# jiwoon-ahn/irn

Hardware: NVIDIA H100
Metric: pseudo-label images/sec (CAM+random-walk) (higher is better)
Workload: dtype f32

## Files before the change

irn_b200/csrc/conv_wgmma.cuh:

```cuda
#pragma once
#include <cuda.h>
#include <cuda_runtime.h>
#include <cstdint>
#include <type_traits>

#include "tma.cuh"

namespace irn {

constexpr int kTcTW = 16, kTcTH = 8;
constexpr int kTcBK = 32;
constexpr int kBfBK = 64;
constexpr int kWgThreads = 384;

struct TcMaps {
    CUtensorMap a;
    CUtensorMap b_hi;
    CUtensorMap b_lo;
    CUtensorMap a2;
};

struct TcArgs {
    const float* bias;
    const float* residual;
    float* out;
    int B, Ho, Wo, Cout, Cin, ksize, stride, pad, relu;
    int tiles_x, tiles_y;
    int kb_split = 1 << 30;
    int stride2 = 1;
    const float* oscale = nullptr;
    int stem = 0;
};

template <bool F16, int BN>
struct WgCfg {
    static constexpr int kBK = F16 ? kBfBK : kTcBK;
    static constexpr int kARaw = F16 ? 32768 : 16384;
    static constexpr int kBBytes = BN * 128;
    static constexpr int kStageBytes = kARaw + 2 * kBBytes;
    static constexpr int kMaxSmem = 227 * 1024;
    static constexpr int kBarBytes = 256;
    static constexpr int kStages = (kMaxSmem - 1024 - kBarBytes) / kStageBytes;
    static constexpr size_t kSmem = 1024 + (size_t)kStages * kStageBytes + kBarBytes;
    static_assert(kStages >= 2, "shared memory holds at least two stages");
    static_assert(2 * kStages * 8 <= kBarBytes, "barrier area holds full[S] and empty[S]");
    static_assert(BN == 64 || BN == 128, "N tile 64 or 128");
};
constexpr int kWgProducerRegs = 40, kWgConsumerRegs = 232;

#ifdef __CUDACC__
__device__ __forceinline__ uint64_t wg_desc(uint32_t smem_addr) {
    return (uint64_t)((smem_addr & 0x3FFFFu) >> 4) | ((uint64_t)1 << 16) | ((uint64_t)(1024 >> 4) << 32) | ((uint64_t)1 << 62);
}
__device__ __forceinline__ void wg_fence() { asm volatile("wgmma.fence.sync.aligned;" ::: "memory"); }
__device__ __forceinline__ void wg_commit() { asm volatile("wgmma.commit_group.sync.aligned;" ::: "memory"); }
template <int N>
__device__ __forceinline__ void wg_wait() { asm volatile("wgmma.wait_group.sync.aligned %0;" ::"n"(N) : "memory"); }
template <int N>
__device__ __forceinline__ void setmaxnreg_inc() { asm volatile("setmaxnreg.inc.sync.aligned.u32 %0;" ::"n"(N)); }
template <int N>
__device__ __forceinline__ void setmaxnreg_dec() { asm volatile("setmaxnreg.dec.sync.aligned.u32 %0;" ::"n"(N)); }
template <int N>
__device__ __forceinline__ void wg_fence_regs(float (&d)[N]) {
#pragma unroll
    for (int i = 0; i < N; ++i) asm volatile("" : "+f"(d[i])::"memory");
}

template <bool F16, int N>
__device__ __forceinline__ void wg_mma(float (&d)[N / 2], const uint32_t (&a)[4], uint64_t db, uint32_t scale_d);

template <> __device__ __forceinline__ void wg_mma<false, 64>(float (&d)[32], const uint32_t (&a)[4], uint64_t db, uint32_t scale_d) {
    asm volatile(
        "{\n\t.reg .pred p;\n\tsetp.ne.b32 p, %37, 0;\n\t"
        "wgmma.mma_async.sync.aligned.m64n64k8.f32.tf32.tf32 {"
        "%0, %1, %2, %3, %4, %5, %6, %7, %8, %9, %10, %11, %12, %13, %14, %15, "
        "%16, %17, %18, %19, %20, %21, %22, %23, %24, %25, %26, %27, %28, %29, %30, %31"
        "}, {%32, %33, %34, %35}, %36, p, 1, 1;\n\t}"
        : "+f"(d[0]), "+f"(d[1]), "+f"(d[2]), "+f"(d[3]), "+f"(d[4]), "+f"(d[5]), "+f"(d[6]), "+f"(d[7]),
          "+f"(d[8]), "+f"(d[9]), "+f"(d[10]), "+f"(d[11]), "+f"(d[12]), "+f"(d[13]), "+f"(d[14]), "+f"(d[15]),
          "+f"(d[16]), "+f"(d[17]), "+f"(d[18]), "+f"(d[19]), "+f"(d[20]), "+f"(d[21]), "+f"(d[22]), "+f"(d[23]),
          "+f"(d[24]), "+f"(d[25]), "+f"(d[26]), "+f"(d[27]), "+f"(d[28]), "+f"(d[29]), "+f"(d[30]), "+f"(d[31])
        : "r"(a[0]), "r"(a[1]), "r"(a[2]), "r"(a[3]), "l"(db), "r"(scale_d));
}

template <> __device__ __forceinline__ void wg_mma<false, 128>(float (&d)[64], const uint32_t (&a)[4], uint64_t db, uint32_t scale_d) {
    asm volatile(
        "{\n\t.reg .pred p;\n\tsetp.ne.b32 p, %69, 0;\n\t"
        "wgmma.mma_async.sync.aligned.m64n128k8.f32.tf32.tf32 {"
        "%0, %1, %2, %3, %4, %5, %6, %7, %8, %9, %10, %11, %12, %13, %14, %15, "
        "%16, %17, %18, %19, %20, %21, %22, %23, %24, %25, %26, %27, %28, %29, %30, %31, "
        "%32, %33, %34, %35, %36, %37, %38, %39, %40, %41, %42, %43, %44, %45, %46, %47, "
        "%48, %49, %50, %51, %52, %53, %54, %55, %56, %57, %58, %59, %60, %61, %62, %63"
        "}, {%64, %65, %66, %67}, %68, p, 1, 1;\n\t}"
        : "+f"(d[0]), "+f"(d[1]), "+f"(d[2]), "+f"(d[3]), "+f"(d[4]), "+f"(d[5]), "+f"(d[6]), "+f"(d[7]),
// ... 11 lines not shown
    asm volatile(
        "{\n\t.reg .pred p;\n\tsetp.ne.b32 p, %37, 0;\n\t"
        "wgmma.mma_async.sync.aligned.m64n64k16.f32.f16.f16 {"
        "%0, %1, %2, %3, %4, %5, %6, %7, %8, %9, %10, %11, %12, %13, %14, %15, "
        "%16, %17, %18, %19, %20, %21, %22, %23, %24, %25, %26, %27, %28, %29, %30, %31"
        "}, {%32, %33, %34, %35}, %36, p, 1, 1, 0;\n\t}"
        : "+f"(d[0]), "+f"(d[1]), "+f"(d[2]), "+f"(d[3]), "+f"(d[4]), "+f"(d[5]), "+f"(d[6]), "+f"(d[7]),
          "+f"(d[8]), "+f"(d[9]), "+f"(d[10]), "+f"(d[11]), "+f"(d[12]), "+f"(d[13]), "+f"(d[14]), "+f"(d[15]),
          "+f"(d[16]), "+f"(d[17]), "+f"(d[18]), "+f"(d[19]), "+f"(d[20]), "+f"(d[21]), "+f"(d[22]), "+f"(d[23]),
          "+f"(d[24]), "+f"(d[25]), "+f"(d[26]), "+f"(d[27]), "+f"(d[28]), "+f"(d[29]), "+f"(d[30]), "+f"(d[31])
        : "r"(a[0]), "r"(a[1]), "r"(a[2]), "r"(a[3]), "l"(db), "r"(scale_d));
}

template <> __device__ __forceinline__ void wg_mma<true, 128>(float (&d)[64], const uint32_t (&a)[4], uint64_t db, uint32_t scale_d) {
    asm volatile(
        "{\n\t.reg .pred p;\n\tsetp.ne.b32 p, %69, 0;\n\t"
        "wgmma.mma_async.sync.aligned.m64n128k16.f32.f16.f16 {"
        "%0, %1, %2, %3, %4, %5, %6, %7, %8, %9, %10, %11, %12, %13, %14, %15, "
        "%16, %17, %18, %19, %20, %21, %22, %23, %24, %25, %26, %27, %28, %29, %30, %31, "
        "%32, %33, %34, %35, %36, %37, %38, %39, %40, %41, %42, %43, %44, %45, %46, %47, "
        "%48, %49, %50, %51, %52, %53, %54, %55, %56, %57, %58, %59, %60, %61, %62, %63"
        "}, {%64, %65, %66, %67}, %68, p, 1, 1, 0;\n\t}"
        : "+f"(d[0]), "+f"(d[1]), "+f"(d[2]), "+f"(d[3]), "+f"(d[4]), "+f"(d[5]), "+f"(d[6]), "+f"(d[7]),
          "+f"(d[8]), "+f"(d[9]), "+f"(d[10]), "+f"(d[11]), "+f"(d[12]), "+f"(d[13]), "+f"(d[14]), "+f"(d[15]),
          "+f"(d[16]), "+f"(d[17]), "+f"(d[18]), "+f"(d[19]), "+f"(d[20]), "+f"(d[21]), "+f"(d[22]), "+f"(d[23]),
          "+f"(d[24]), "+f"(d[25]), "+f"(d[26]), "+f"(d[27]), "+f"(d[28]), "+f"(d[29]), "+f"(d[30]), "+f"(d[31]),
          "+f"(d[32]), "+f"(d[33]), "+f"(d[34]), "+f"(d[35]), "+f"(d[36]), "+f"(d[37]), "+f"(d[38]), "+f"(d[39]),
          "+f"(d[40]), "+f"(d[41]), "+f"(d[42]), "+f"(d[43]), "+f"(d[44]), "+f"(d[45]), "+f"(d[46]), "+f"(d[47]),
          "+f"(d[48]), "+f"(d[49]), "+f"(d[50]), "+f"(d[51]), "+f"(d[52]), "+f"(d[53]), "+f"(d[54]), "+f"(d[55]),
          "+f"(d[56]), "+f"(d[57]), "+f"(d[58]), "+f"(d[59]), "+f"(d[60]), "+f"(d[61]), "+f"(d[62]), "+f"(d[63])
        : "r"(a[0]), "r"(a[1]), "r"(a[2]), "r"(a[3]), "l"(db), "r"(scale_d));
}

__device__ __forceinline__ float tf32_hi(float x) { return __uint_as_float((__float_as_uint(x) + 0x1000u) & 0xFFFFE000u); }

__device__ __forceinline__ void f16_split2(float a, float b, uint32_t& hi, uint32_t& lo) {
    asm("cvt.rz.satfinite.f16x2.f32 %0, %1, %2;" : "=r"(hi) : "f"(b), "f"(a));
    const float ha = __uint_as_float(__float_as_uint(a) & 0xFFFFE000u), hb = __uint_as_float(__float_as_uint(b) & 0xFFFFE000u);
    asm("cvt.rn.satfinite.f16x2.f32 %0, %1, %2;" : "=r"(lo) : "f"(b - hb), "f"(a - ha));
}

template <bool F16>
__device__ __forceinline__ void wg_load_frag(const unsigned char* row, int k, int key, int t4, float (&v)[8]) {
    if (F16) {
        const unsigned char* box = row + (k >> 1) * 16384;
        const int c = 4 * (k & 1) + (t4 >> 1);
        const float2 x0 = *reinterpret_cast<const float2*>(box + ((c ^ key) << 4));
        const float2 x1 = *reinterpret_cast<const float2*>(box + 1024 + ((c ^ key) << 4));
        const float2 x2 = *reinterpret_cast<const float2*>(box + (((c + 2) ^ key) << 4));
        const float2 x3 = *reinterpret_cast<const float2*>(box + 1024 + (((c + 2) ^ key) << 4));
        v[0] = x0.x; v[1] = x0.y; v[2] = x1.x; v[3] = x1.y; v[4] = x2.x; v[5] = x2.y; v[6] = x3.x; v[7] = x3.y;
    } else {
        const int c = 2 * k;
        v[0] = *reinterpret_cast<const float*>(row + ((c ^ key) << 4));
        v[1] = *reinterpret_cast<const float*>(row + 1024 + ((c ^ key) << 4));
        v[2] = *reinterpret_cast<const float*>(row + (((c + 1) ^ key) << 4));
        v[3] = *reinterpret_cast<const float*>(row + 1024 + (((c + 1) ^ key) << 4));
    }
}

template <bool F16>
__device__ __forceinline__ void wg_split_frag(const float (&v)[8], uint32_t (&hi)[4], uint32_t (&lo)[4]) {
#pragma unroll
    for (int i = 0; i < 4; ++i) {
        if (F16) {
            f16_split2(v[2 * i], v[2 * i + 1], hi[i], lo[i]);
        } else {
            const float h = tf32_hi(v[i]);
            hi[i] = __float_as_uint(h);
            lo[i] = __float_as_uint(v[i] - h);
        }
    }
}

template <bool F16, int BN>
__global__ void __launch_bounds__(kWgThreads, 1)
conv_wg_kernel(const __grid_constant__ TcMaps maps, const TcArgs args) {
    using Cfg = WgCfg<F16, BN>;
    constexpr int S = Cfg::kStages;
    constexpr int R = BN / 2;
    extern __shared__ unsigned char wg_smem_raw[];
    unsigned char* smem = wg_smem_raw + ((1024u - (smem_u32(wg_smem_raw) & 1023u)) & 1023u);
    uint64_t* bars = (uint64_t*)(smem + S * Cfg::kStageBytes);
    uint64_t* full = bars;
    uint64_t* empty = bars + S;

    const int warp = threadIdx.x >> 5, lane = threadIdx.x & 31;
    const int n_tiles = args.Cout / BN;
    const int n_items = args.tiles_x * args.tiles_y * args.B * n_tiles;
    const int cblocks = args.Cin / Cfg::kBK;
    const int KB = (!F16 && args.stem) ? args.ksize : args.ksize * args.ksize * cblocks;

    if (threadIdx.x == 0) {
        for (int s = 0; s < S; ++s) {
            mbar_init(&full[s], 1);
            mbar_init(&empty[s], 8);
        }
        fence_mbar_init();
    }
    __syncthreads();

    if (warp < 4) {
        setmaxnreg_dec<kWgProducerRegs>();
        if (threadIdx.x == 0) {
            tma_prefetch_desc(&maps.a);
            tma_prefetch_desc(&maps.b_hi);
            tma_prefetch_desc(&maps.b_lo);
            if (F16 && args.kb_split < KB) tma_prefetch_desc(&maps.a2);
            int s = 0;
            uint32_t ph = 0;
            for (int item = blockIdx.x; item < n_items; item += gridDim.x) {
                const int tile = item / n_tiles;
                const int ox0 = (tile % args.tiles_x) * kTcTW;
                const int oy0 = ((tile / args.tiles_x) % args.tiles_y) * kTcTH;
                const int b = tile / (args.tiles_x * args.tiles_y);
                const int n0 = (item % n_tiles) * BN;
                for (int kb = 0; kb < KB; ++kb) {
                    mbar_wait(&empty[s], ph ^ 1);
                    unsigned char* st = smem + s * Cfg::kStageBytes;
                    unsigned char* wb = st + Cfg::kARaw;
                    mbar_arrive_expect_tx(&full[s], (uint32_t)Cfg::kStageBytes);
                    if (args.stem) {
                        const int row = F16 ? 2 * kb : kb;
                        tma_load_4d(st, &maps.a, &full[s], 0, ox0, oy0 * 2 + row, b);
                        if (F16) tma_load_4d(st + 16384, &maps.a, &full[s], 0, ox0, oy0 * 2 + row + 1, b);
                    } else {
                        const bool second = F16 && kb >= args.kb_split;
                        const CUtensorMap* am = second ? &maps.a2 : &maps.a;
                        const int tap = second ? 0 : kb / cblocks, cb = second ? kb - args.kb_split : kb % cblocks;
                        const int r = tap / args.ksize, ss = tap % args.ksize;
                        const int x = second ? ox0 * args.stride2 : ox0 * args.stride - args.pad + ss;
                        const int y = second ? oy0 * args.stride2 : oy0 * args.stride - args.pad + r;
                        tma_load_4d(st, am, &full[s], cb * Cfg::kBK, x, y, b);
                        if (F16) tma_load_4d(st + 16384, am, &full[s], cb * Cfg::kBK + 32, x, y, b);
                    }
                    tma_load_2d(wb, &maps.b_hi, &full[s], kb * Cfg::kBK, n0);
                    tma_load_2d(wb + Cfg::kBBytes, &maps.b_lo, &full[s], kb * Cfg::kBK, n0);
                    if (++s == S) { s = 0; ph ^= 1; }
                }
            }
        }
        return;
    }

    setmaxnreg_inc<kWgConsumerRegs>();
    const int g = (threadIdx.x >> 7) - 1, wq = warp & 3;
    const int key = lane >> 2, t4 = lane & 3;
    const int frag_off = (64 * g + 16 * wq + key) * 128 + (F16 ? 8 * (t4 & 1) : 4 * t4);
    float acc[R], part[2][R];
    uint32_t fa[2][2][4];
    int s = 0, s_prev = 0;
    uint32_t ph = 0;
    auto promote = [&](auto P) {
        constexpr int p = decltype(P)::value;
        wg_fence_regs(part[p]);
#pragma unroll
        for (int i = 0; i < R; ++i) acc[i] += part[p][i];
        __syncwarp();
        if (lane == 0) mbar_arrive(&empty[s_prev]);
    };
    auto kblock = [&](auto P) {
        constexpr int p = decltype(P)::value;
        mbar_wait(&full[s], ph);
        unsigned char* st = smem + s * Cfg::kStageBytes;
        const unsigned char* frag = st + frag_off;
        const uint32_t b_hi = smem_u32(st + Cfg::kARaw), b_lo = b_hi + Cfg::kBBytes;
#pragma unroll
        for (int k = 0; k < 4; ++k) {
            float v[8];
            wg_load_frag<F16>(frag, k, key, t4, v);
            wg_wait<1>();
            if (p == 1 && k == 1) promote(std::integral_constant<int, 0>());
            wg_split_frag<F16>(v, fa[k & 1][0], fa[k & 1][1]);
            if (k == 0) wg_fence_regs(part[p]);
            wg_fence();
            const uint64_t db_hi = wg_desc(b_hi + 32 * k), db_lo = wg_desc(b_lo + 32 * k);
            wg_mma<F16, BN>(part[p], fa[k & 1][0], db_hi, k != 0 ? 1u : 0u);
            wg_mma<F16, BN>(part[p], fa[k & 1][1], db_hi, 1u);
            wg_mma<F16, BN>(part[p], fa[k & 1][0], db_lo, 1u);
            wg_commit();
        }
        s_prev = s;
        if (++s == S) { s = 0; ph ^= 1; }
    };

    for (int item = blockIdx.x; item < n_items; item += gridDim.x) {
        const int tile = item / n_tiles;
        const int ox0 = (tile % args.tiles_x) * kTcTW;
        const int oy0 = ((tile / args.tiles_x) % args.tiles_y) * kTcTH;
        const int b = tile / (args.tiles_x * args.tiles_y);
        const int n0 = (item % n_tiles) * BN;
#pragma unroll
        for (int i = 0; i < R; ++i) acc[i] = 0.f;
        int kb = 0;
        for (; kb + 1 < KB; kb += 2) {
            kblock(std::integral_constant<int, 0>());
            kblock(std::integral_constant<int, 1>());
            wg_wait<0>();
            promote(std::integral_constant<int, 1>());
        }
        if (kb < KB) {
            kblock(std::integral_constant<int, 0>());
            wg_wait<0>();
            promote(std::integral_constant<int, 0>());
        }

#pragma unroll
        for (int h = 0; h < 2; ++h) {
            const int row = 64 * g + 16 * wq + (lane >> 2) + 8 * h;
            const int oy = oy0 + row / kTcTW, ox = ox0 + row % kTcTW;
            if (oy >= args.Ho || ox >= args.Wo) continue;
            const size_t base = (((size_t)b * args.Ho + oy) * args.Wo + ox) * args.Cout + n0 + 2 * (lane & 3);
#pragma unroll
            for (int j = 0; j < BN / 8; ++j) {
                const int n = n0 + 8 * j + 2 * (lane & 3);
                float2 o = make_float2(acc[4 * j + 2 * h], acc[4 * j + 2 * h + 1]);
                if (F16 && args.oscale) {
                    const float2 sc = __ldg(reinterpret_cast<const float2*>(args.oscale + n));
                    o.x *= sc.x; o.y *= sc.y;
                }
                if (args.bias) {
                    const float2 bi = __ldg(reinterpret_cast<const float2*>(args.bias + n));
                    o.x += bi.x; o.y += bi.y;
                }
                if (args.residual) {
                    const float2 rv = __ldg(reinterpret_cast<const float2*>(args.residual + base + 8 * j));
                    o.x += rv.x; o.y += rv.y;
                }
                if (args.relu) {
                    o.x = fmaxf(o.x, 0.f); o.y = fmaxf(o.y, 0.f);
                }
                *reinterpret_cast<float2*>(args.out + base + 8 * j) = o;
            }
        }
    }
}
#endif

}
```

irn_b200/csrc/nets.cu:

```cuda
#include <cuda_fp16.h>

#include <cmath>
#include <cstdlib>
#include <cstring>
#include <vector>

#include "common.h"
#include "conv_simt.cuh"
#include "conv_wgmma.cuh"

namespace irn {

struct Conv {
    int cin = 0, cout = 0, k = 1, stride = 1, pad = 0;
    float* wt = nullptr;
    float* bias = nullptr;
    float* w_hi = nullptr;
    float* w_lo = nullptr;
    int bn = 0;
    CUtensorMap map_bhi, map_blo;
    uint16_t* wb_hi = nullptr;
    uint16_t* wb_lo = nullptr;
    float* oscale = nullptr;
    bool bf_ok = false;
// ... 98 lines not shown
    if ((rc = make_bf16_weights(net, c, wt))) return rc;
    c.bn = (cout % 128 == 0) ? 128 : (cout % 64 == 0 ? 64 : 0);
    if (cin % kTcBK != 0 || !(k == 1 || k == 3) || !(stride == 1 || stride == 2)) c.bn = 0;
    if (c.bn) {
        const size_t K = (size_t)k * k * cin;
        std::vector<float> hi(nw), lo(nw);
        for (int o = 0; o < cout; ++o)
            for (size_t kk = 0; kk < K; ++kk) {
                const float v = wt[kk * cout + o];
                uint32_t u;
                std::memcpy(&u, &v, 4);
                uint32_t h = (u + 0x1000u) & 0xFFFFE000u;
                float hf;
                std::memcpy(&hf, &h, 4);
                if (!std::isfinite(hf)) hf = v;
                hi[(size_t)o * K + kk] = hf;
                lo[(size_t)o * K + kk] = v - hf;
            }
        if ((rc = upload(net, hi, &c.w_hi))) return rc;
        if ((rc = upload(net, lo, &c.w_lo))) return rc;
        const uint64_t dims[2] = {(uint64_t)K, (uint64_t)cout};
        const uint64_t strides[1] = {(uint64_t)K * sizeof(float)};
        const uint32_t box[2] = {(uint32_t)kTcBK, (uint32_t)c.bn};
        if ((rc = make_tensor_map(&c.map_bhi, CU_TENSOR_MAP_DATA_TYPE_FLOAT32, 2, c.w_hi, dims, strides, box, CU_TENSOR_MAP_SWIZZLE_128B))) return rc;
        if ((rc = make_tensor_map(&c.map_blo, CU_TENSOR_MAP_DATA_TYPE_FLOAT32, 2, c.w_lo, dims, strides, box, CU_TENSOR_MAP_SWIZZLE_128B))) return rc;
    }
    return kOk;
}

static int make_bf16_weights(irn_net* net, Conv& c, const std::vector<float>& wt ) {
    const size_t K = (size_t)c.k * c.k * c.cin;
    c.bf_ok = c.cin % kBfBK == 0 && c.cout % 64 == 0 && (c.k == 1 || c.k == 3) && (c.stride == 1 || c.stride == 2);
    if (!c.bf_ok) return kOk;
    std::vector<uint16_t> hi((size_t)c.cout * K), lo((size_t)c.cout * K);
    std::vector<float> inv(c.cout, 1.0f);
    for (int o = 0; o < c.cout; ++o) {
        float mx = 0.f;
        for (size_t kk = 0; kk < K; ++kk) mx = std::max(mx, std::fabs(wt[kk * c.cout + o]));
        int e = 1;
        if (mx > 0.f && std::isfinite(mx)) std::frexp(mx, &e);
        const int sh = 1 - e;
        inv[o] = std::ldexp(1.0f, -sh);
        for (size_t kk = 0; kk < K; ++kk) {
            const float v = std::ldexp(wt[kk * c.cout + o], sh);
            const __half h = __float2half_rn(v);
            const __half l = __float2half_rn(v - __half2float(h));
            hi[(size_t)o * K + kk] = __half_as_ushort(h);
            lo[(size_t)o * K + kk] = __half_as_ushort(l);
        }
    }
    int rc = upload(net, inv, &c.oscale);
    if (rc) return rc;
    for (int part = 0; part < 2; ++part) {
        void* d = nullptr;
        IRN_CUDA(cudaMalloc(&d, hi.size() * sizeof(uint16_t)));
        net->allocs.push_back(d);
        IRN_CUDA(cudaMemcpy(d, part == 0 ? hi.data() : lo.data(), hi.size() * sizeof(uint16_t), cudaMemcpyHostToDevice));
        (part == 0 ? c.wb_hi : c.wb_lo) = (uint16_t*)d;
    }
    const uint64_t dims[2] = {(uint64_t)K, (uint64_t)c.cout};
    const uint64_t strides[1] = {(uint64_t)K * sizeof(uint16_t)};
    for (int i = 0; i < 2; ++i) {
        const uint32_t rows = 64u << i;
        if (c.cout % rows != 0) continue;
        const uint32_t box[2] = {(uint32_t)kBfBK, rows};
        if ((rc = make_tensor_map(&c.map_bf_hi[i], CU_TENSOR_MAP_DATA_TYPE_FLOAT16, 2, c.wb_hi, dims, strides, box, CU_TENSOR_MAP_SWIZZLE_128B))) return rc;
        if ((rc = make_tensor_map(&c.map_bf_lo[i], CU_TENSOR_MAP_DATA_TYPE_FLOAT16, 2, c.wb_lo, dims, strides, box, CU_TENSOR_MAP_SWIZZLE_128B))) return rc;
    }
    return kOk;
}

static int read_vec(irn_net* net, Reader& rd, size_t n, float** out) {
    const float* p = rd.take(n);
    if (!rd.ok) return fail(kBadArg, "parameter blob too short (vector of %zu)", n);
    return upload(net, std::vector<float>(p, p + n), out);
}

static int read_trunk(irn_net* net, Reader& rd) {
    int rc = read_conv(net, rd, net->stem, 3, 64, 7, 2, 3, true);
    if (rc) return rc;
    {
// ... 52 lines not shown
                f.cin = K3 + Kd; f.cout = cout; f.k = 1; f.stride = 1; f.pad = 0;
                std::vector<float> wt((size_t)(K3 + Kd) * cout), bias(cout);
                std::copy(blk.c3.host_wt.begin(), blk.c3.host_wt.end(), wt.begin());
                std::copy(blk.ds.host_wt.begin(), blk.ds.host_wt.end(), wt.begin() + (size_t)K3 * cout);
                for (int o = 0; o < cout; ++o) bias[o] = blk.c3.host_bias[o] + blk.ds.host_bias[o];
                if ((rc = upload(net, bias, &f.bias))) return rc;
                if ((rc = make_bf16_weights(net, f, wt))) return rc;
                blk.has_c3ds = f.bf_ok;
            }
            cin = planes * 4;
        }
    }
    net->stem.host_wt.clear(); net->stem.host_wt.shrink_to_fit();
    for (int l = 0; l < 4; ++l)
        for (Block& blk : net->blocks[l])
            for (Conv* c : {&blk.c1, &blk.c2, &blk.c3, &blk.ds}) {
                std::vector<float>().swap(c->host_wt);
                std::vector<float>().swap(c->host_bias);
            }
    return kOk;
}

static int read_head(irn_net* net, Reader& rd, Head& h, int cin, int cout, int groups, int up) {
    int rc = read_conv(net, rd, h.conv, cin, cout, 1, 1, 0, false);
    if (rc) return rc;
    h.groups = groups;
    h.up = up;
    if ((rc = read_vec(net, rd, cout, &h.gamma))) return rc;
    return read_vec(net, rd, cout, &h.beta);
}

static inline int conv_out(int n, int k, int s, int p) { return (n + 2 * p - k) / s + 1; }

template <bool F16, int BN>
static int launch_wg(const TcMaps& maps, const TcArgs& a, cudaStream_t st) {
    using Cfg = WgCfg<F16, BN>;
    static DeviceOnce once;
    const int ds = once.slot();
    if (once.need(ds)) {
        IRN_CUDA(cudaFuncSetAttribute((conv_wg_kernel<F16, BN>), cudaFuncAttributeMaxDynamicSharedMemorySize, (int)Cfg::kSmem));
        int dev = 0, n_sm = 0, per_sm = 0;
        IRN_CUDA(cudaGetDevice(&dev));
        IRN_CUDA(cudaDeviceGetAttribute(&n_sm, cudaDevAttrMultiProcessorCount, dev));
        IRN_CUDA(cudaOccupancyMaxActiveBlocksPerMultiprocessor(&per_sm, conv_wg_kernel<F16, BN>, kWgThreads, Cfg::kSmem));
        if (per_sm < 1) return fail(kCudaError, "conv_wg_kernel: no CTA fits on an SM (%zu bytes of shared memory)", Cfg::kSmem);
        once.n_sm[ds] = n_sm * per_sm;
        once.done[ds] = true;
    }
    const long long items = (long long)a.tiles_x * a.tiles_y * a.B * (a.Cout / BN);
    const long long grid = items < once.n_sm[ds] ? items : once.n_sm[ds];
    conv_wg_kernel<F16, BN><<<(unsigned)grid, kWgThreads, Cfg::kSmem, st>>>(maps, a);
    IRN_LAUNCH_CHECK(F16 ? "conv_wg_kernel<f16x3>" : "conv_wg_kernel<3xtf32>");
    return kOk;
}

static TcArgs conv_args(const Conv& c, int B, int Ho, int Wo, const float* residual, float* out, bool relu) {
    TcArgs a;
    a.bias = c.bias; a.residual = residual; a.out = out;
    a.oscale = c.oscale;
    a.B = B; a.Ho = Ho; a.Wo = Wo; a.Cout = c.cout; a.Cin = c.cin; a.ksize = c.k; a.stride = c.stride; a.pad = c.pad;
    a.relu = relu ? 1 : 0;
    a.tiles_x = (Wo + kTcTW - 1) / kTcTW;
    a.tiles_y = (Ho + kTcTH - 1) / kTcTH;
    return a;
}

static int act_map(CUtensorMap* m, const float* in, int B, int H, int W, int cin, int stride) {
    const uint64_t dims[4] = {(uint64_t)cin, (uint64_t)W, (uint64_t)H, (uint64_t)B};
    const uint64_t strides[3] = {(uint64_t)cin * 4, (uint64_t)W * cin * 4, (uint64_t)H * W * cin * 4};
    const uint32_t box[4] = {32u, (uint32_t)(kTcTW * stride), (uint32_t)(kTcTH * stride), 1};
    const uint32_t estr[4] = {1, (uint32_t)stride, (uint32_t)stride, 1};
    return make_tensor_map(m, CU_TENSOR_MAP_DATA_TYPE_FLOAT32, 4, in, dims, strides, box, CU_TENSOR_MAP_SWIZZLE_128B, estr);
}

static int stem_map(CUtensorMap* m, const float* x4, int B, int Hin, int Win) {
    const int Hp = Hin + 6, Wp = Win + 8;
    const int Wo = conv_out(Win, 7, 2, 3);
    const uint64_t dims[4] = {32, (uint64_t)Wo, (uint64_t)Hp, (uint64_t)B};
    const uint64_t strides[3] = {32, (uint64_t)Wp * 16, (uint64_t)Hp * Wp * 16};
    const uint32_t box[4] = {32, (uint32_t)kTcTW, (uint32_t)(kTcTH * 2), 1};
    const uint32_t estr[4] = {1, 1, 2, 1};
    return make_tensor_map(m, CU_TENSOR_MAP_DATA_TYPE_FLOAT32, 4, x4, dims, strides, box, CU_TENSOR_MAP_SWIZZLE_128B, estr);
}

static int run_conv_tf32(const Conv& c, const float* in, int B, int H, int W, int Ho, int Wo, const float* residual, float* out, bool relu,
                         cudaStream_t st) {
    TcMaps maps;
    maps.b_hi = c.map_bhi;
    maps.b_lo = c.map_blo;
    int rc = act_map(&maps.a, in, B, H, W, c.cin, c.stride);
    if (rc) return rc;
    maps.a2 = maps.a;
    TcArgs a = conv_args(c, B, Ho, Wo, residual, out, relu);
    a.oscale = nullptr;
    return c.bn == 128 ? launch_wg<false, 128>(maps, a, st) : launch_wg<false, 64>(maps, a, st);
}

static int launch_tf32_stem(const Conv& c, const float* x4, int B, int Hin, int Win, float* out, cudaStream_t st) {
    TcMaps maps;
    maps.b_hi = c.map_bhi;
    maps.b_lo = c.map_blo;
    int rc = stem_map(&maps.a, x4, B, Hin, Win);
    if (rc) return rc;
    maps.a2 = maps.a;
    TcArgs a = conv_args(c, B, conv_out(Hin, 7, 2, 3), conv_out(Win, 7, 2, 3), nullptr, out, true);
    a.oscale = nullptr;
    a.Cin = 32; a.ksize = 7; a.stride = 2; a.pad = 3; a.stem = 1;
    return launch_wg<false, 64>(maps, a, st);
}

struct F16Second {
    const float* in = nullptr;
    int H = 0, W = 0, cin = 0, stride = 1;
};

static int run_conv_f16(const Conv& c, const float* in, int B, int H, int W, int Ho, int Wo, const float* residual, float* out, bool relu,
                        cudaStream_t st, const F16Second* second = nullptr) {
    const bool wide = c.cout % 128 == 0;
    TcMaps maps;
    maps.b_hi = c.map_bf_hi[wide ? 1 : 0];
    maps.b_lo = c.map_bf_lo[wide ? 1 : 0];
    const int cin1 = second ? c.cin - second->cin : c.cin;
    int rc = act_map(&maps.a, in, B, H, W, cin1, c.stride);
    if (rc) return rc;
    maps.a2 = maps.a;
    TcArgs a = conv_args(c, B, Ho, Wo, residual, out, relu);
    if (second) {
        if (c.k != 1) return fail(kUnsupported, "run_conv_f16: a second input needs a 1x1 conv");
        if ((rc = act_map(&maps.a2, second->in, B, second->H, second->W, second->cin, second->stride))) return rc;
        a.kb_split = cin1 / kBfBK;
        a.stride2 = second->stride;
    }
    return wide ? launch_wg<true, 128>(maps, a, st) : launch_wg<true, 64>(maps, a, st);
}

static int launch_f16_stem(const Conv& c, const float* x4, int B, int Hin, int Win, float* out, cudaStream_t st) {
    TcMaps maps;
    maps.b_hi = c.map_bf_hi[0];
    maps.b_lo = c.map_bf_lo[0];
    int rc = stem_map(&maps.a, x4, B, Hin, Win);
    if (rc) return rc;
    maps.a2 = maps.a;
    TcArgs a = conv_args(c, B, conv_out(Hin, 7, 2, 3), conv_out(Win, 7, 2, 3), nullptr, out, true);
    a.Cin = 256; a.ksize = 1; a.stride = 2; a.pad = 0; a.stem = 1;
    return launch_wg<true, 64>(maps, a, st);
}

static int run_conv(const irn_net* net, const Conv& c, const float* in, int B, int H, int W, const float* residual, float* out, bool relu,
                    cudaStream_t st, int* Ho_, int* Wo_) {
    ConvGeom g;
    g.B = B; g.H = H; g.W = W; g.Cin = c.cin;
    g.Ho = conv_out(H, c.k, c.stride, c.pad);
    g.Wo = conv_out(W, c.k, c.stride, c.pad);
    g.Cout = c.cout; g.k = c.k; g.stride = c.stride; g.pad = c.pad;
// ... 361 lines not shown
```

irn_b200/csrc/tma.cuh:

```cuda
#pragma once
#include <cuda.h>
#include <cuda_runtime.h>
#include <cstdint>

#include "common.h"

namespace irn {

typedef CUresult (*EncodeTiledFn)(CUtensorMap*, CUtensorMapDataType, cuuint32_t, void*, const cuuint64_t*,
                                  const cuuint64_t*, const cuuint32_t*, const cuuint32_t*, CUtensorMapInterleave,
                                  CUtensorMapSwizzle, CUtensorMapL2promotion, CUtensorMapFloatOOBfill);

inline EncodeTiledFn encode_tiled_fn() {
    static EncodeTiledFn fn = nullptr;
    if (!fn) {
        void* p = nullptr;
        cudaDriverEntryPointQueryResult q;
        if (cudaGetDriverEntryPoint("cuTensorMapEncodeTiled", &p, cudaEnableDefault, &q) == cudaSuccess &&
            q == cudaDriverEntryPointSuccess)
            fn = (EncodeTiledFn)p;
    }
    return fn;
}

// ... 60 lines not shown
        : "r"(smem_u32(bar)), "r"(parity)
        : "memory");
    return ok != 0;
}
__device__ __forceinline__ void mbar_wait_spin(uint64_t* bar, uint32_t parity) {
    for (uint32_t spin = 0; !mbar_test_wait(bar, parity); ++spin)
        if (spin > (1u << 28)) __trap();
}

__device__ __forceinline__ void tma_load_3d(void* smem_dst, const CUtensorMap* map, uint64_t* bar, int c0, int c1, int c2) {
    asm volatile(
        "cp.async.bulk.tensor.3d.shared::cluster.global.mbarrier::complete_tx::bytes [%0], [%1, {%3, %4, %5}], [%2];"
        ::"r"(smem_u32(smem_dst)), "l"(map), "r"(smem_u32(bar)), "r"(c0), "r"(c1), "r"(c2)
        : "memory");
}
__device__ __forceinline__ void tma_load_4d(void* smem_dst, const CUtensorMap* map, uint64_t* bar, int c0, int c1, int c2, int c3) {
    asm volatile(
        "cp.async.bulk.tensor.4d.shared::cluster.global.mbarrier::complete_tx::bytes [%0], [%1, {%3, %4, %5, %6}], [%2];"
        ::"r"(smem_u32(smem_dst)), "l"(map), "r"(smem_u32(bar)), "r"(c0), "r"(c1), "r"(c2), "r"(c3)
        : "memory");
}
__device__ __forceinline__ void tma_load_2d(void* smem_dst, const CUtensorMap* map, uint64_t* bar, int c0, int c1) {
    asm volatile(
        "cp.async.bulk.tensor.2d.shared::cluster.global.mbarrier::complete_tx::bytes [%0], [%1, {%3, %4}], [%2];"
        ::"r"(smem_u32(smem_dst)), "l"(map), "r"(smem_u32(bar)), "r"(c0), "r"(c1)
        : "memory");
}
__device__ __forceinline__ void tma_prefetch_3d(const CUtensorMap* map, int c0, int c1, int c2) {
    asm volatile("cp.async.bulk.prefetch.tensor.3d.L2.global.tile [%0, {%1, %2, %3}];" ::"l"(map), "r"(c0), "r"(c1), "r"(c2) : "memory");
}
__device__ __forceinline__ void tma_prefetch_desc(const CUtensorMap* map) {
    asm volatile("prefetch.tensormap [%0];" ::"l"(map) : "memory");
}
#endif

}
```

Before: 91.86.

## Load a halo activation tile once per channel block for 3x3 stride-1 convs

For 3x3 stride-1 f16x3 convolutions, the producer now loads one (TH+2)x(TW+2) halo tile per 64-channel block into two dedicated double-buffered slots. The consumers read all nine taps from that tile by shifting row offsets, where before each tap fetched its own activation box by TMA. Weights are reordered on the host so the nine taps of a channel block are contiguous, matching the new k-loop order. The consumer loop is also unrolled into longer runs (4 or 2 k-blocks) between promotions. This cuts activation traffic roughly ninefold and frees ring space for B stages, at the cost of added barrier and indexing complexity.

```diff
diff --git a/irn_b200/csrc/conv_wgmma.cuh b/irn_b200/csrc/conv_wgmma.cuh
--- a/irn_b200/csrc/conv_wgmma.cuh
+++ b/irn_b200/csrc/conv_wgmma.cuh
@@ -32,19 +32,26 @@
     int stem = 0;
 };
 
-template <bool F16, int BN>
+template <bool F16, int BN, bool HALO = false>
 struct WgCfg {
     static constexpr int kBK = F16 ? kBfBK : kTcBK;
-    static constexpr int kARaw = F16 ? 32768 : 16384;
+    static constexpr int kHaloRows = (kTcTH + 2) * (kTcTW + 2);
+    static constexpr int kAHalo = kHaloRows * 128;
+    static constexpr int kABox = HALO ? (kAHalo + 1023) / 1024 * 1024 : 16384;
+    static constexpr int kASlots = HALO ? 2 : 0;
+    static constexpr int kASlot = 2 * kABox;
+    static constexpr int kARaw = HALO ? 0 : (F16 ? 32768 : 16384);
     static constexpr int kBBytes = BN * 128;
     static constexpr int kStageBytes = kARaw + 2 * kBBytes;
     static constexpr int kMaxSmem = 227 * 1024;
     static constexpr int kBarBytes = 256;
-    static constexpr int kStages = (kMaxSmem - 1024 - kBarBytes) / kStageBytes;
-    static constexpr size_t kSmem = 1024 + (size_t)kStages * kStageBytes + kBarBytes;
+    static constexpr int kStages = (kMaxSmem - 1024 - kBarBytes - kASlots * kASlot) / kStageBytes;
+    static constexpr size_t kSmem = 1024 + (size_t)kASlots * kASlot + (size_t)kStages * kStageBytes + kBarBytes;
     static_assert(kStages >= 2, "shared memory holds at least two stages");
-    static_assert(2 * kStages * 8 <= kBarBytes, "barrier area holds full[S] and empty[S]");
+    static_assert(kSmem <= (size_t)kMaxSmem, "shared-memory plan fits 227 KB");
+    static_assert((2 * kStages + 2 * kASlots) * 8 <= kBarBytes, "barrier area holds every mbarrier");
     static_assert(BN == 64 || BN == 128, "N tile 64 or 128");
+    static_assert(!HALO || F16, "the halo tile is an f16x3 (64-channel k-block) plan");
 };
 constexpr int kWgProducerRegs = 40, kWgConsumerRegs = 232;
 
@@ -137,6 +144,14 @@
         : "r"(a[0]), "r"(a[1]), "r"(a[2]), "r"(a[3]), "l"(db), "r"(scale_d));
 }
 
+template <int I, int N, class F>
+__device__ __forceinline__ void wg_static_for(F& f) {
+    if constexpr (I < N) {
+        f(std::integral_constant<int, I>());
+        wg_static_for<I + 1, N>(f);
+    }
+}
+
 __device__ __forceinline__ float tf32_hi(float x) { return __uint_as_float((__float_as_uint(x) + 0x1000u) & 0xFFFFE000u); }
 
 __device__ __forceinline__ void f16_split2(float a, float b, uint32_t& hi, uint32_t& lo) {
@@ -145,10 +160,10 @@
     asm("cvt.rn.satfinite.f16x2.f32 %0, %1, %2;" : "=r"(lo) : "f"(b - hb), "f"(a - ha));
 }
 
-template <bool F16>
+template <bool F16, int kBox>
 __device__ __forceinline__ void wg_load_frag(const unsigned char* row, int k, int key, int t4, float (&v)[8]) {
     if (F16) {
-        const unsigned char* box = row + (k >> 1) * 16384;
+        const unsigned char* box = row + (k >> 1) * kBox;
         const int c = 4 * (k & 1) + (t4 >> 1);
         const float2 x0 = *reinterpret_cast<const float2*>(box + ((c ^ key) << 4));
         const float2 x1 = *reinterpret_cast<const float2*>(box + 1024 + ((c ^ key) << 4));
@@ -178,17 +193,20 @@
     }
 }
 
-template <bool F16, int BN>
+template <bool F16, int BN, bool HALO = false>
 __global__ void __launch_bounds__(kWgThreads, 1)
 conv_wg_kernel(const __grid_constant__ TcMaps maps, const TcArgs args) {
-    using Cfg = WgCfg<F16, BN>;
+    using Cfg = WgCfg<F16, BN, HALO>;
     constexpr int S = Cfg::kStages;
     constexpr int R = BN / 2;
     extern __shared__ unsigned char wg_smem_raw[];
     unsigned char* smem = wg_smem_raw + ((1024u - (smem_u32(wg_smem_raw) & 1023u)) & 1023u);
-    uint64_t* bars = (uint64_t*)(smem + S * Cfg::kStageBytes);
+    unsigned char* ring = smem + Cfg::kASlots * Cfg::kASlot;
+    uint64_t* bars = (uint64_t*)(ring + S * Cfg::kStageBytes);
     uint64_t* full = bars;
     uint64_t* empty = bars + S;
+    uint64_t* a_full = bars + 2 * S;
+    uint64_t* a_empty = bars + 2 * S + 2;
 
     const int warp = threadIdx.x >> 5, lane = threadIdx.x & 31;
     const int n_tiles = args.Cout / BN;
@@ -200,6 +218,10 @@
         for (int s = 0; s < S; ++s) {
             mbar_init(&full[s], 1);
             mbar_init(&empty[s], 8);
+        }
+        for (int s = 0; s < Cfg::kASlots; ++s) {
+            mbar_init(&a_full[s], 1);
+            mbar_init(&a_empty[s], 8);
         }
         fence_mbar_init();
     }
@@ -212,8 +234,8 @@
             tma_prefetch_desc(&maps.b_hi);
             tma_prefetch_desc(&maps.b_lo);
             if (F16 && args.kb_split < KB) tma_prefetch_desc(&maps.a2);
-            int s = 0;
-            uint32_t ph = 0;
+            int s = 0, as = 0;
+            uint32_t ph = 0, aph = 0;
             for (int item = blockIdx.x; item < n_items; item += gridDim.x) {
                 const int tile = item / n_tiles;
                 const int ox0 = (tile % args.tiles_x) * kTcTW;
@@ -221,11 +243,21 @@
                 const int b = tile / (args.tiles_x * args.tiles_y);
                 const int n0 = (item % n_tiles) * BN;
                 for (int kb = 0; kb < KB; ++kb) {
+                    if (HALO && kb % 9 == 0) {
+                        mbar_wait(&a_empty[as], aph ^ 1);
+                        unsigned char* at = smem + as * Cfg::kASlot;
+                        const int c0 = (kb / 9) * Cfg::kBK;
+                        mbar_arrive_expect_tx(&a_full[as], 2u * Cfg::kAHalo);
+                        tma_load_4d(at, &maps.a, &a_full[as], c0, ox0 - args.pad, oy0 - args.pad, b);
+                        tma_load_4d(at + Cfg::kABox, &maps.a, &a_full[as], c0 + 32, ox0 - args.pad, oy0 - args.pad, b);
+                        if (++as == 2) { as = 0; aph ^= 1; }
+                    }
                     mbar_wait(&empty[s], ph ^ 1);
-                    unsigned char* st = smem + s * Cfg::kStageBytes;
+                    unsigned char* st = ring + s * Cfg::kStageBytes;
                     unsigned char* wb = st + Cfg::kARaw;
                     mbar_arrive_expect_tx(&full[s], (uint32_t)Cfg::kStageBytes);
-                    if (args.stem) {
+                    if (HALO) {
+                    } else if (args.stem) {
                         const int row = F16 ? 2 * kb : kb;
                         tma_load_4d(st, &maps.a, &full[s], 0, ox0, oy0 * 2 + row, b);
                         if (F16) tma_load_4d(st + 16384, &maps.a, &full[s], 0, ox0, oy0 * 2 + row + 1, b);
@@ -252,30 +284,44 @@
     const int g = (threadIdx.x >> 7) - 1, wq = warp & 3;
     const int key = lane >> 2, t4 = lane & 3;
     const int frag_off = (64 * g + 16 * wq + key) * 128 + (F16 ? 8 * (t4 & 1) : 4 * t4);
+    const int hrow = (4 * g + wq) * (kTcTW + 2) + key;
+    constexpr int kRun = BN == 64 ? 4 : 2;
     float acc[R], part[2][R];
     uint32_t fa[2][2][4];
     int s = 0, s_prev = 0;
     uint32_t ph = 0;
+    int as = 0, tap = 0, a_prev = -1;
+    uint32_t aph = 0;
     auto promote = [&](auto P) {
         constexpr int p = decltype(P)::value;
         wg_fence_regs(part[p]);
 #pragma unroll
         for (int i = 0; i < R; ++i) acc[i] += part[p][i];
         __syncwarp();
-        if (lane == 0) mbar_arrive(&empty[s_prev]);
+        if (lane == 0) {
+            mbar_arrive(&empty[s_prev]);
+            if (HALO && a_prev >= 0) mbar_arrive(&a_empty[a_prev]);
+        }
     };
-    auto kblock = [&](auto P) {
-        constexpr int p = decltype(P)::value;
+    auto kblock = [&](auto J) {
+        constexpr int j = decltype(J)::value, p = j & 1;
+        unsigned char* st = ring + s * Cfg::kStageBytes;
+        const unsigned char* frag = st + frag_off;
+        int fkey = key;
+        if (HALO) {
+            if (tap == 0) mbar_wait(&a_full[as], aph);
+            const int i = hrow + tap + 15 * (tap / 3);
+            frag = smem + as * Cfg::kASlot + i * 128 + 8 * (t4 & 1);
+            fkey = i & 7;
+        }
         mbar_wait(&full[s], ph);
-        unsigned char* st = smem + s * Cfg::kStageBytes;
-        const unsigned char* frag = st + frag_off;
         const uint32_t b_hi = smem_u32(st + Cfg::kARaw), b_lo = b_hi + Cfg::kBBytes;
 #pragma unroll
         for (int k = 0; k < 4; ++k) {
             float v[8];
-            wg_load_frag<F16>(frag, k, key, t4, v);
+            wg_load_frag<F16, Cfg::kABox>(frag, k, fkey, t4, v);
             wg_wait<1>();
-            if (p == 1 && k == 1) promote(std::integral_constant<int, 0>());
+            if (j > 0 && k == 1) promote(std::integral_constant<int, p ^ 1>());
             wg_split_frag<F16>(v, fa[k & 1][0], fa[k & 1][1]);
             if (k == 0) wg_fence_regs(part[p]);
             wg_fence();
@@ -287,6 +333,19 @@
         }
         s_prev = s;
         if (++s == S) { s = 0; ph ^= 1; }
+        if (HALO) {
+            a_prev = tap == 8 ? as : -1;
+            if (++tap == 9) {
+                tap = 0;
+                if (++as == 2) { as = 0; aph ^= 1; }
+            }
+        }
+    };
+    auto run = [&](auto N) {
+        constexpr int n = decltype(N)::value;
+        wg_static_for<0, n>(kblock);
+        wg_wait<0>();
+        promote(std::integral_constant<int, (n - 1) & 1>());
     };
 
     for (int item = blockIdx.x; item < n_items; item += gridDim.x) {
@@ -298,17 +357,11 @@
 #pragma unroll
         for (int i = 0; i < R; ++i) acc[i] = 0.f;
         int kb = 0;
-        for (; kb + 1 < KB; kb += 2) {
-            kblock(std::integral_constant<int, 0>());
-            kblock(std::integral_constant<int, 1>());
-            wg_wait<0>();
-            promote(std::integral_constant<int, 1>());
-        }
-        if (kb < KB) {
-            kblock(std::integral_constant<int, 0>());
-            wg_wait<0>();
-            promote(std::integral_constant<int, 0>());
-        }
+        for (; kb + kRun <= KB; kb += kRun) run(std::integral_constant<int, kRun>());
+        if constexpr (kRun > 2) {
+            if (KB - kb >= 2) { run(std::integral_constant<int, 2>()); kb += 2; }
+        }
+        if (kb < KB) run(std::integral_constant<int, 1>());
 
 #pragma unroll
         for (int h = 0; h < 2; ++h) {
diff --git a/irn_b200/csrc/nets.cu b/irn_b200/csrc/nets.cu
--- a/irn_b200/csrc/nets.cu
+++ b/irn_b200/csrc/nets.cu
@@ -154,6 +154,7 @@
     const size_t K = (size_t)c.k * c.k * c.cin;
     c.bf_ok = c.cin % kBfBK == 0 && c.cout % 64 == 0 && (c.k == 1 || c.k == 3) && (c.stride == 1 || c.stride == 2);
     if (!c.bf_ok) return kOk;
+    const bool halo = c.k == 3 && c.stride == 1;
     std::vector<uint16_t> hi((size_t)c.cout * K), lo((size_t)c.cout * K);
     std::vector<float> inv(c.cout, 1.0f);
     for (int o = 0; o < c.cout; ++o) {
@@ -167,8 +168,10 @@
             const float v = std::ldexp(wt[kk * c.cout + o], sh);
             const __half h = __float2half_rn(v);
             const __half l = __float2half_rn(v - __half2float(h));
-            hi[(size_t)o * K + kk] = __half_as_ushort(h);
-            lo[(size_t)o * K + kk] = __half_as_ushort(l);
+            const size_t tap = kk / c.cin, ci = kk % c.cin;
+            const size_t kp = halo ? ((ci / kBfBK) * 9 + tap) * kBfBK + ci % kBfBK : kk;
+            hi[(size_t)o * K + kp] = __half_as_ushort(h);
+            lo[(size_t)o * K + kp] = __half_as_ushort(l);
         }
     }
     int rc = upload(net, inv, &c.oscale);
@@ -287,25 +290,25 @@
 
 static inline int conv_out(int n, int k, int s, int p) { return (n + 2 * p - k) / s + 1; }
 
-template <bool F16, int BN>
+template <bool F16, int BN, bool HALO = false>
 static int launch_wg(const TcMaps& maps, const TcArgs& a, cudaStream_t st) {
-    using Cfg = WgCfg<F16, BN>;
+    using Cfg = WgCfg<F16, BN, HALO>;
     static DeviceOnce once;
     const int ds = once.slot();
     if (once.need(ds)) {
-        IRN_CUDA(cudaFuncSetAttribute((conv_wg_kernel<F16, BN>), cudaFuncAttributeMaxDynamicSharedMemorySize, (int)Cfg::kSmem));
+        IRN_CUDA(cudaFuncSetAttribute((conv_wg_kernel<F16, BN, HALO>), cudaFuncAttributeMaxDynamicSharedMemorySize, (int)Cfg::kSmem));
         int dev = 0, n_sm = 0, per_sm = 0;
         IRN_CUDA(cudaGetDevice(&dev));
         IRN_CUDA(cudaDeviceGetAttribute(&n_sm, cudaDevAttrMultiProcessorCount, dev));
-        IRN_CUDA(cudaOccupancyMaxActiveBlocksPerMultiprocessor(&per_sm, conv_wg_kernel<F16, BN>, kWgThreads, Cfg::kSmem));
+        IRN_CUDA(cudaOccupancyMaxActiveBlocksPerMultiprocessor(&per_sm, conv_wg_kernel<F16, BN, HALO>, kWgThreads, Cfg::kSmem));
         if (per_sm < 1) return fail(kCudaError, "conv_wg_kernel: no CTA fits on an SM (%zu bytes of shared memory)", Cfg::kSmem);
         once.n_sm[ds] = n_sm * per_sm;
         once.done[ds] = true;
     }
     const long long items = (long long)a.tiles_x * a.tiles_y * a.B * (a.Cout / BN);
     const long long grid = items < once.n_sm[ds] ? items : once.n_sm[ds];
-    conv_wg_kernel<F16, BN><<<(unsigned)grid, kWgThreads, Cfg::kSmem, st>>>(maps, a);
-    IRN_LAUNCH_CHECK(F16 ? "conv_wg_kernel<f16x3>" : "conv_wg_kernel<3xtf32>");
+    conv_wg_kernel<F16, BN, HALO><<<(unsigned)grid, kWgThreads, Cfg::kSmem, st>>>(maps, a);
+    IRN_LAUNCH_CHECK(HALO ? "conv_wg_kernel<f16x3, halo>" : F16 ? "conv_wg_kernel<f16x3>" : "conv_wg_kernel<3xtf32>");
     return kOk;
 }
 
@@ -328,6 +331,14 @@
     return make_tensor_map(m, CU_TENSOR_MAP_DATA_TYPE_FLOAT32, 4, in, dims, strides, box, CU_TENSOR_MAP_SWIZZLE_128B, estr);
 }
 
+static int halo_map(CUtensorMap* m, const float* in, int B, int H, int W, int cin) {
+    const uint64_t dims[4] = {(uint64_t)cin, (uint64_t)W, (uint64_t)H, (uint64_t)B};
+    const uint64_t strides[3] = {(uint64_t)cin * 4, (uint64_t)W * cin * 4, (uint64_t)H * W * cin * 4};
+    const uint32_t box[4] = {32u, (uint32_t)(kTcTW + 2), (uint32_t)(kTcTH + 2), 1};
+    const uint32_t estr[4] = {1, 1, 1, 1};
+    return make_tensor_map(m, CU_TENSOR_MAP_DATA_TYPE_FLOAT32, 4, in, dims, strides, box, CU_TENSOR_MAP_SWIZZLE_128B, estr);
+}
+
 static int stem_map(CUtensorMap* m, const float* x4, int B, int Hin, int Win) {
     const int Hp = Hin + 6, Wp = Win + 8;
     const int Wo = conv_out(Win, 7, 2, 3);
@@ -375,6 +386,14 @@
     TcMaps maps;
     maps.b_hi = c.map_bf_hi[wide ? 1 : 0];
     maps.b_lo = c.map_bf_lo[wide ? 1 : 0];
+    if (c.k == 3 && c.stride == 1) {
+        if (second) return fail(kUnsupported, "run_conv_f16: a second input needs a 1x1 conv");
+        int rc = halo_map(&maps.a, in, B, H, W, c.cin);
+        if (rc) return rc;
+        maps.a2 = maps.a;
+        const TcArgs a = conv_args(c, B, Ho, Wo, residual, out, relu);
+        return wide ? launch_wg<true, 128, true>(maps, a, st) : launch_wg<true, 64, true>(maps, a, st);
+    }
     const int cin1 = second ? c.cin - second->cin : c.cin;
     int rc = act_map(&maps.a, in, B, H, W, cin1, c.stride);
     if (rc) return rc;
```

Result: faster. 93.72 (median of 6 runs) (+2.0%).

## Stage conv epilogue through swizzled shared memory and store with TMA

Applied to the files above, without the earlier changes.

Adds a STAGED variant of the wgmma conv kernel. When there is no residual input, consumers write the bias, scale and relu results into a 128B-swizzled shared buffer, then one thread issues TMA tensor stores in 64-channel chunks. This replaces scattered float2 global stores with bulk async stores that can overlap the next tile's main loop. The cost is 32KB of shared memory taken from the pipeline stages, which may drop one stage, plus extra named-barrier syncs in the epilogue.

```diff
diff --git a/irn_b200/csrc/conv_wgmma.cuh b/irn_b200/csrc/conv_wgmma.cuh
--- a/irn_b200/csrc/conv_wgmma.cuh
+++ b/irn_b200/csrc/conv_wgmma.cuh
@@ -18,6 +18,7 @@
     CUtensorMap b_hi;
     CUtensorMap b_lo;
     CUtensorMap a2;
+    CUtensorMap out;
 };
 
 struct TcArgs {
@@ -32,18 +33,19 @@
     int stem = 0;
 };
 
-template <bool F16, int BN>
+template <bool F16, int BN, bool STAGED>
 struct WgCfg {
     static constexpr int kBK = F16 ? kBfBK : kTcBK;
     static constexpr int kARaw = F16 ? 32768 : 16384;
     static constexpr int kBBytes = BN * 128;
     static constexpr int kStageBytes = kARaw + 2 * kBBytes;
     static constexpr int kMaxSmem = 227 * 1024;
+    static constexpr int kOutBytes = STAGED ? 32768 : 0;
     static constexpr int kBarBytes = 256;
-    static constexpr int kStages = (kMaxSmem - 1024 - kBarBytes) / kStageBytes;
-    static constexpr size_t kSmem = 1024 + (size_t)kStages * kStageBytes + kBarBytes;
+    static constexpr int kStages = (kMaxSmem - 1024 - kOutBytes - kBarBytes) / kStageBytes;
+    static constexpr size_t kSmem = 1024 + (size_t)kStages * kStageBytes + kOutBytes + kBarBytes;
     static_assert(kStages >= 2, "shared memory holds at least two stages");
-    static_assert(2 * kStages * 8 <= kBarBytes, "barrier area holds full[S] and empty[S]");
+    static_assert(2 * kStages * 8 <= 128, "barrier area holds full[S] and empty[S] below the store slot");
     static_assert(BN == 64 || BN == 128, "N tile 64 or 128");
 };
 constexpr int kWgProducerRegs = 40, kWgConsumerRegs = 232;
@@ -60,6 +62,7 @@
 __device__ __forceinline__ void setmaxnreg_inc() { asm volatile("setmaxnreg.inc.sync.aligned.u32 %0;" ::"n"(N)); }
 template <int N>
 __device__ __forceinline__ void setmaxnreg_dec() { asm volatile("setmaxnreg.dec.sync.aligned.u32 %0;" ::"n"(N)); }
+__device__ __forceinline__ void consumer_sync() { asm volatile("bar.sync 1, 256;" ::: "memory"); }
 template <int N>
 __device__ __forceinline__ void wg_fence_regs(float (&d)[N]) {
 #pragma unroll
@@ -178,17 +181,40 @@
     }
 }
 
-template <bool F16, int BN>
+template <bool F16, int R>
+__device__ __forceinline__ float2 wg_epi_value(const TcArgs& args, const float (&acc)[R], int j, int h, int n, size_t roff, bool inside) {
+    float2 o = make_float2(acc[4 * j + 2 * h], acc[4 * j + 2 * h + 1]);
+    if (F16 && args.oscale) {
+        const float2 sc = __ldg(reinterpret_cast<const float2*>(args.oscale + n));
+        o.x *= sc.x; o.y *= sc.y;
+    }
+    if (args.bias) {
+        const float2 bi = __ldg(reinterpret_cast<const float2*>(args.bias + n));
+        o.x += bi.x; o.y += bi.y;
+    }
+    if (args.residual && inside) {
+        const float2 rv = __ldg(reinterpret_cast<const float2*>(args.residual + roff));
+        o.x += rv.x; o.y += rv.y;
+    }
+    if (args.relu) {
+        o.x = fmaxf(o.x, 0.f); o.y = fmaxf(o.y, 0.f);
+    }
+    return o;
+}
+
+template <bool F16, int BN, bool STAGED>
 __global__ void __launch_bounds__(kWgThreads, 1)
 conv_wg_kernel(const __grid_constant__ TcMaps maps, const TcArgs args) {
-    using Cfg = WgCfg<F16, BN>;
+    using Cfg = WgCfg<F16, BN, STAGED>;
     constexpr int S = Cfg::kStages;
     constexpr int R = BN / 2;
     extern __shared__ unsigned char wg_smem_raw[];
     unsigned char* smem = wg_smem_raw + ((1024u - (smem_u32(wg_smem_raw) & 1023u)) & 1023u);
-    uint64_t* bars = (uint64_t*)(smem + S * Cfg::kStageBytes);
+    unsigned char* stage_out = smem + S * Cfg::kStageBytes;
+    uint64_t* bars = (uint64_t*)(stage_out + Cfg::kOutBytes);
     uint64_t* full = bars;
     uint64_t* empty = bars + S;
+    volatile int* store_slot = reinterpret_cast<volatile int*>(bars + 16);
 
     const int warp = threadIdx.x >> 5, lane = threadIdx.x & 31;
     const int n_tiles = args.Cout / BN;
@@ -212,6 +238,7 @@
             tma_prefetch_desc(&maps.b_hi);
             tma_prefetch_desc(&maps.b_lo);
             if (F16 && args.kb_split < KB) tma_prefetch_desc(&maps.a2);
+            if (STAGED) tma_prefetch_desc(&maps.out);
             int s = 0;
             uint32_t ph = 0;
             for (int item = blockIdx.x; item < n_items; item += gridDim.x) {
@@ -295,6 +322,10 @@
         const int oy0 = ((tile / args.tiles_x) % args.tiles_y) * kTcTH;
         const int b = tile / (args.tiles_x * args.tiles_y);
         const int n0 = (item % n_tiles) * BN;
+        if (STAGED && threadIdx.x == 128) {
+            store_slot[0] = n0; store_slot[1] = ox0; store_slot[2] = oy0; store_slot[3] = b;
+            store_slot[4] = item + (int)gridDim.x >= n_items;
+        }
 #pragma unroll
         for (int i = 0; i < R; ++i) acc[i] = 0.f;
         int kb = 0;
@@ -310,32 +341,45 @@
             promote(std::integral_constant<int, 0>());
         }
 
-#pragma unroll
-        for (int h = 0; h < 2; ++h) {
-            const int row = 64 * g + 16 * wq + (lane >> 2) + 8 * h;
-            const int oy = oy0 + row / kTcTW, ox = ox0 + row % kTcTW;
-            if (oy >= args.Ho || ox >= args.Wo) continue;
-            const size_t base = (((size_t)b * args.Ho + oy) * args.Wo + ox) * args.Cout + n0 + 2 * (lane & 3);
-#pragma unroll
-            for (int j = 0; j < BN / 8; ++j) {
-                const int n = n0 + 8 * j + 2 * (lane & 3);
-                float2 o = make_float2(acc[4 * j + 2 * h], acc[4 * j + 2 * h + 1]);
-                if (F16 && args.oscale) {
-                    const float2 sc = __ldg(reinterpret_cast<const float2*>(args.oscale + n));
-                    o.x *= sc.x; o.y *= sc.y;
+        if constexpr (!STAGED) {
+#pragma unroll
+            for (int h = 0; h < 2; ++h) {
+                const int row = 64 * g + 16 * wq + key + 8 * h;
+                const int oy = oy0 + row / kTcTW, ox = ox0 + row % kTcTW;
+                if (oy >= args.Ho || ox >= args.Wo) continue;
+                const size_t base = (((size_t)b * args.Ho + oy) * args.Wo + ox) * args.Cout + n0 + 2 * t4;
+#pragma unroll
+                for (int j = 0; j < BN / 8; ++j)
+                    *reinterpret_cast<float2*>(args.out + base + 8 * j) = wg_epi_value<F16>(args, acc, j, h, n0 + 8 * j + 2 * t4, base + 8 * j, true);
+            }
+        } else {
+#pragma unroll
+            for (int q = 0; q < BN / 64; ++q) {
+                if (threadIdx.x == 128) bulk_wait_read<0>();
+                consumer_sync();
+#pragma unroll
+                for (int h = 0; h < 2; ++h) {
+                    const int row = 64 * g + 16 * wq + key + 8 * h;
+                    const int oy = oy0 + row / kTcTW, ox = ox0 + row % kTcTW;
+                    const bool inside = oy < args.Ho && ox < args.Wo;
+                    const size_t base = (((size_t)b * args.Ho + oy) * args.Wo + ox) * args.Cout + n0 + 2 * t4;
+                    unsigned char* dst = stage_out + row * 128 + 8 * (t4 & 1);
+#pragma unroll
+                    for (int jj = 0; jj < 8; ++jj) {
+                        const int j = 8 * q + jj;
+                        *reinterpret_cast<float2*>(dst + (jj >> 2) * 16384 + (((2 * (jj & 3) + (t4 >> 1)) ^ key) << 4)) =
+                            wg_epi_value<F16>(args, acc, j, h, n0 + 8 * j + 2 * t4, base + 8 * j, inside);
+                    }
                 }
-                if (args.bias) {
-                    const float2 bi = __ldg(reinterpret_cast<const float2*>(args.bias + n));
-                    o.x += bi.x; o.y += bi.y;
+                fence_proxy_async();
+                consumer_sync();
+                if (threadIdx.x == 128) {
+                    const int c0 = store_slot[0] + 64 * q, c1 = store_slot[1], c2 = store_slot[2], c3 = store_slot[3];
+                    tma_store_4d(&maps.out, stage_out, c0, c1, c2, c3);
+                    tma_store_4d(&maps.out, stage_out + 16384, c0 + 32, c1, c2, c3);
+                    bulk_commit();
+                    if (q == BN / 64 - 1 && store_slot[4]) bulk_wait<0>();
                 }
-                if (args.residual) {
-                    const float2 rv = __ldg(reinterpret_cast<const float2*>(args.residual + base + 8 * j));
-                    o.x += rv.x; o.y += rv.y;
-                }
-                if (args.relu) {
-                    o.x = fmaxf(o.x, 0.f); o.y = fmaxf(o.y, 0.f);
-                }
-                *reinterpret_cast<float2*>(args.out + base + 8 * j) = o;
             }
         }
     }
diff --git a/irn_b200/csrc/nets.cu b/irn_b200/csrc/nets.cu
--- a/irn_b200/csrc/nets.cu
+++ b/irn_b200/csrc/nets.cu
@@ -287,26 +287,39 @@
 
 static inline int conv_out(int n, int k, int s, int p) { return (n + 2 * p - k) / s + 1; }
 
-template <bool F16, int BN>
-static int launch_wg(const TcMaps& maps, const TcArgs& a, cudaStream_t st) {
-    using Cfg = WgCfg<F16, BN>;
+template <bool F16, int BN, bool STAGED>
+static int launch_wg_as(const TcMaps& maps, const TcArgs& a, cudaStream_t st) {
+    using Cfg = WgCfg<F16, BN, STAGED>;
     static DeviceOnce once;
     const int ds = once.slot();
     if (once.need(ds)) {
-        IRN_CUDA(cudaFuncSetAttribute((conv_wg_kernel<F16, BN>), cudaFuncAttributeMaxDynamicSharedMemorySize, (int)Cfg::kSmem));
+        IRN_CUDA(cudaFuncSetAttribute((conv_wg_kernel<F16, BN, STAGED>), cudaFuncAttributeMaxDynamicSharedMemorySize, (int)Cfg::kSmem));
         int dev = 0, n_sm = 0, per_sm = 0;
         IRN_CUDA(cudaGetDevice(&dev));
         IRN_CUDA(cudaDeviceGetAttribute(&n_sm, cudaDevAttrMultiProcessorCount, dev));
-        IRN_CUDA(cudaOccupancyMaxActiveBlocksPerMultiprocessor(&per_sm, conv_wg_kernel<F16, BN>, kWgThreads, Cfg::kSmem));
+        IRN_CUDA(cudaOccupancyMaxActiveBlocksPerMultiprocessor(&per_sm, conv_wg_kernel<F16, BN, STAGED>, kWgThreads, Cfg::kSmem));
         if (per_sm < 1) return fail(kCudaError, "conv_wg_kernel: no CTA fits on an SM (%zu bytes of shared memory)", Cfg::kSmem);
         once.n_sm[ds] = n_sm * per_sm;
         once.done[ds] = true;
     }
     const long long items = (long long)a.tiles_x * a.tiles_y * a.B * (a.Cout / BN);
     const long long grid = items < once.n_sm[ds] ? items : once.n_sm[ds];
-    conv_wg_kernel<F16, BN><<<(unsigned)grid, kWgThreads, Cfg::kSmem, st>>>(maps, a);
+    conv_wg_kernel<F16, BN, STAGED><<<(unsigned)grid, kWgThreads, Cfg::kSmem, st>>>(maps, a);
     IRN_LAUNCH_CHECK(F16 ? "conv_wg_kernel<f16x3>" : "conv_wg_kernel<3xtf32>");
     return kOk;
+}
+
+template <bool F16, int BN>
+static int launch_wg(TcMaps maps, const TcArgs& a, cudaStream_t st) {
+    const int KB = (!F16 && a.stem) ? a.ksize : a.ksize * a.ksize * (a.Cin / WgCfg<F16, BN, false>::kBK);
+    maps.out = maps.a;
+    if (a.residual || KB < 2) return launch_wg_as<F16, BN, false>(maps, a, st);
+    const uint64_t dims[4] = {(uint64_t)a.Cout, (uint64_t)a.Wo, (uint64_t)a.Ho, (uint64_t)a.B};
+    const uint64_t strides[3] = {(uint64_t)a.Cout * 4, (uint64_t)a.Wo * a.Cout * 4, (uint64_t)a.Ho * a.Wo * a.Cout * 4};
+    const uint32_t box[4] = {32u, (uint32_t)kTcTW, (uint32_t)kTcTH, 1u};
+    const int rc = make_tensor_map(&maps.out, CU_TENSOR_MAP_DATA_TYPE_FLOAT32, 4, a.out, dims, strides, box, CU_TENSOR_MAP_SWIZZLE_128B);
+    if (rc) return rc;
+    return launch_wg_as<F16, BN, true>(maps, a, st);
 }
 
 static TcArgs conv_args(const Conv& c, int B, int Ho, int Wo, const float* residual, float* out, bool relu) {
diff --git a/irn_b200/csrc/tma.cuh b/irn_b200/csrc/tma.cuh
--- a/irn_b200/csrc/tma.cuh
+++ b/irn_b200/csrc/tma.cuh
@@ -116,6 +116,16 @@
 __device__ __forceinline__ void tma_prefetch_desc(const CUtensorMap* map) {
     asm volatile("prefetch.tensormap [%0];" ::"l"(map) : "memory");
 }
+__device__ __forceinline__ void tma_store_4d(const CUtensorMap* map, const void* smem_src, int c0, int c1, int c2, int c3) {
+    asm volatile("cp.async.bulk.tensor.4d.global.shared::cta.bulk_group [%0, {%2, %3, %4, %5}], [%1];"
+                 ::"l"(map), "r"(smem_u32(smem_src)), "r"(c0), "r"(c1), "r"(c2), "r"(c3)
+                 : "memory");
+}
+__device__ __forceinline__ void bulk_commit() { asm volatile("cp.async.bulk.commit_group;" ::: "memory"); }
+template <int N>
+__device__ __forceinline__ void bulk_wait_read() { asm volatile("cp.async.bulk.wait_group.read %0;" ::"n"(N) : "memory"); }
+template <int N>
+__device__ __forceinline__ void bulk_wait() { asm volatile("cp.async.bulk.wait_group %0;" ::"n"(N) : "memory"); }
 #endif
 
 }
```

After: 91.33 before, 93.28 after, median of 6. 1.02x the previous value.
